# dropbox/rust-brotli

Measured on AMD Instinct MI355X. Metric: compress MB/s at q5 lgwin22, higher is better.
Workload: dtype u8; 1 GPU; 64 MiB synthetic English-like text per GPU, quality=5, lgwin=22, one-shot BrotliEncoderCompress (H6), input and stream resident in HBM; input_bytes_total=67108864, compressed_bytes=16370400

## Files before the change

### rust-brotli_amd/csrc/encoder.cpp

```cpp
#include "encoder.h"
#include "timeline.h"

#include <math.h>
#include <string.h>

#include <algorithm>
#include <chrono>
#include <stdexcept>

#include "device_api.h"
#include "host_entropy.h"
#include "lz77_stage.h"
#include "metablock_api.h"
#include "metablock_device.h"
#include "metablock_hq.h"
#include "metablock_items.h"

namespace brotli_mi355x {

namespace {

struct DevMem {
  DevBlocks blocks;
  static constexpr size_t kArenaBytes = (size_t)4 << 20, kSmall = (size_t)256 << 10;
  uint8_t* arena = nullptr;
  size_t arena_used = kArenaBytes;
  template <typename T>
  T* alloc(size_t count) {
    const size_t bytes = (count * sizeof(T) + 64 + 255) & ~(size_t)255;
    if (bytes > kSmall) return blocks.zeroed<T>(bytes);
    if (arena_used + bytes > kArenaBytes) {
      arena = blocks.zeroed<uint8_t>(kArenaBytes);
      arena_used = 0;
    }
    T* p = (T*)(arena + arena_used);
    arena_used += bytes;
    return p;
  }
};

struct BitPiece {
  uint64_t pos;
  uint32_t nbits;
  uint32_t pad;
  uint64_t bits;
};

struct HostBits {
  uint64_t pos = 0;
  std::vector<BitPiece> pieces;
  void put(uint32_t nbits, uint64_t bits) {
    if (nbits == 0) return;
    pieces.push_back({pos, nbits, 0, bits});
    pos += nbits;
  }
  void jump_to_byte_boundary() { pos = (pos + 7) & ~(uint64_t)7; }
};

void WriteMetadataMetaBlock(const EncoderParams& p, HostBits* hb) {
  uint8_t b128[10];
  size_t count = 0;
  uint64_t value = p.size_hint;
  for (size_t index = 0; index < 10; ++index) {
    b128[index] = (uint8_t)(value & 0x7f);
    value >>= 7;
    count = index + 1;
    if (value != 0) {
      b128[index] |= 0x80;
    } else {
      break;
    }
  }
// ... 640 lines not shown
          j.out_cost = mm.alloc<float>(n + 2);
          j.cluster_size = mm.alloc<uint32_t>(n + 8);
          j.clusters = mm.alloc<uint32_t>(n + 8);
          j.symbols = mm.alloc<uint32_t>(n + 8);
          j.new_index = mm.alloc<uint32_t>(n + 8);
          j.batch_count = mm.alloc<uint32_t>(n / kHqBatch + 8);
          j.reindex_data = mm.alloc<uint32_t>(re * j.len + 8);
          j.reindex_total = mm.alloc<uint32_t>(re + 8);
          j.reindex_cost = mm.alloc<float>(re + 8);
          j.pairs = mm.alloc<HqPair>(std::max<size_t>(kHqBatchPairs, 64 * n) + 2);
          cjobs.push_back(j);
        }
      }
      dev_h2d(B.descs, descs.data(), n_mb * sizeof(MbDesc));
      mb_hq_context_histograms(B);
      HqClusterJob* cjobs_dev = mm.alloc<HqClusterJob>(cjobs.size() + 1);
      dev_h2d(cjobs_dev, cjobs.data(), cjobs.size() * sizeof(HqClusterJob));
      std::vector<HqBatchRef> cbatch_refs;
      for (uint32_t ji = 0; ji < cjobs.size(); ++ji)
        for (uint32_t b = 0; b * kHqBatch < cjobs[ji].in_size; ++b) cbatch_refs.push_back({ji, b});
      HqBatchRef* cbatch_refs_dev = mm.alloc<HqBatchRef>(cbatch_refs.size() + 1);
      dev_h2d(cbatch_refs_dev, cbatch_refs.data(), cbatch_refs.size() * sizeof(HqBatchRef));
      mb_hq_cluster_histograms(B, cjobs_dev, (uint32_t)cjobs.size(), cbatch_refs_dev, (uint32_t)cbatch_refs.size());
      dev_d2h(results.data(), B.results, n_mb * sizeof(MbResult));
      for (uint32_t m = 0; m < n_mb; ++m) results[m].num_histos[kSplitCommand] = results[m].num_types[kSplitCommand];
      dev_h2d(B.results, results.data(), n_mb * sizeof(MbResult));
      stats.ms_phase[3] += clk.lap(prof, "hq-context-maps");
    } else {
      if (p.disable_literal_context_modeling == 0 && p.quality >= 5) {
        uint32_t* stats_dev = mm.alloc<uint32_t>((size_t)n_mb * kContextStatsWords);
        mb_context_stats(B, stats_dev);
        std::vector<uint32_t> cs((size_t)n_mb * kContextStatsWords);
        dev_d2h(cs.data(), stats_dev, cs.size() * 4);
        for (uint32_t m = 0; m < n_mb; ++m) {
          if (descs[m].uncompressed) continue;
          DecideContexts(cs.data() + (size_t)m * kContextStatsWords, p.quality, p.size_hint, descs[m].end - descs[m].start,
                         &descs[m].num_contexts, &descs[m].context_map_id);
        }
      }
      uint32_t gran_total[3] = {0, 0, 0}, row_total[3] = {0, 0, 0}, block_total[3] = {0, 0, 0}, histo_total[3] = {0, 0, 0};
      for (uint32_t m = 0; m < n_mb; ++m) {
        MbDesc& d = descs[m];
        d.n_symbols[0] = d.n_lits;
        d.n_symbols[1] = d.n_cmds;
        d.n_symbols[2] = d.n_dists;
        for (uint32_t k = 0; k < 3; ++k) {
          const uint32_t gl = kGranuleLen[k];
          const uint32_t nc = k == 0 ? d.num_contexts : 1;
          d.granule_base[k] = gran_total[k];
          d.n_granules[k] = d.uncompressed ? 0 : (d.n_symbols[k] + gl - 1) / gl;
          d.gran_row_base[k] = row_total[k];
          d.block_base[k] = block_total[k];
          d.max_blocks[k] = d.n_symbols[k] / gl + 1;
          const uint32_t max_types = (k == 0 && nc > 1) ? 256 / nc : 256;
          d.histo_base[k] = histo_total[k];
          d.max_histos[k] = std::min(d.max_blocks[k], max_types + 1) * nc;
          gran_total[k] += d.n_granules[k];
          row_total[k] += d.n_granules[k] * nc;
          block_total[k] += d.max_blocks[k] + 1;
          histo_total[k] += d.max_histos[k];
        }
      }
      std::vector<uint32_t> gran_mb_host[3];
      for (uint32_t k = 0; k < 3; ++k) {
        gran_mb_host[k].resize(gran_total[k] + 1);
        for (uint32_t m = 0; m < n_mb; ++m)
// ... 72 lines not shown
        if (is_last) {
          bits.put(1, 1);
          bits.put(1, 1);
          bits.jump_to_byte_boundary();
        }
      } else {
        const uint64_t start_bit = bits.pos;
        mb_out_bit[m] = start_bit;
        const uint64_t body_bits = body_off[m + 1] - body_off[m];
        bits.pos += results[m].header_bits + body_bits;
        if (is_last) bits.jump_to_byte_boundary();
        if ((uint64_t)bytes + 4 + (start_bit >> 3) < (bits.pos >> 3)) {
          fallback = (int)m;
          break;
        }
      }
      if (actual_last != is_last) WriteEmptyLastBlocks(p, &bits);
    }
    if (fallback >= 0) {
      lz.ForceUncompressed((uint32_t)fallback);
      stats.fallback_retries++;
      continue;
    }
    if (req.finish && lz.needs_empty_last()) WriteEmptyLastBlocks(p, &bits);
    if (!req.finish && !partial) WriteOpenTail(req, &bits);
    const size_t all_bytes = (size_t)((bits.pos + 7) >> 3);
    const uint32_t tail_nbits = partial ? (uint32_t)(bits.pos & 7) : 0u;
    const size_t total_bytes = tail_nbits ? all_bytes - 1 : all_bytes;
    const size_t out_words = all_bytes / 8 + 4;
    B.out_words = mm.alloc<uint64_t>(out_words);
    if (!all_raw) {
      dev_h2d(B.mb_out_bit, mb_out_bit.data(), (n_mb + 1) * 8);
      mb_emit(B);
    }
    {
      std::vector<MbBitCopy> headers;
      for (uint32_t m = 0; m < n_mb; ++m)
        if (!descs[m].uncompressed) headers.push_back({mb_out_bit[m], (uint64_t)m * B.header_stride, results[m].header_bits});
      std::vector<MbRawCopy> raws;
      for (const RawCopy& rc : copies) raws.push_back({rc.dst_byte, rc.src_pos, rc.bytes});
      std::vector<MbBitPiece> pieces;
      for (const BitPiece& bp : bits.pieces) pieces.push_back({bp.pos, bp.nbits, 0, bp.bits});
      const size_t bytes = headers.size() * sizeof(MbBitCopy) + raws.size() * sizeof(MbRawCopy) + pieces.size() * sizeof(MbBitPiece);
      if (bytes != 0) {
        std::vector<uint8_t> blob(bytes);
        uint8_t* at = blob.data();
        memcpy(at, headers.data(), headers.size() * sizeof(MbBitCopy));
        at += headers.size() * sizeof(MbBitCopy);
        memcpy(at, raws.data(), raws.size() * sizeof(MbRawCopy));
        at += raws.size() * sizeof(MbRawCopy);
        memcpy(at, pieces.data(), pieces.size() * sizeof(MbBitPiece));
        uint8_t* blob_dev = mm.alloc<uint8_t>(bytes + 64);
        dev_h2d(blob_dev, blob.data(), bytes);
        const MbBitCopy* headers_dev = (const MbBitCopy*)blob_dev;
        const MbRawCopy* raws_dev = (const MbRawCopy*)(blob_dev + headers.size() * sizeof(MbBitCopy));
        const MbBitPiece* pieces_dev = (const MbBitPiece*)(blob_dev + headers.size() * sizeof(MbBitCopy) + raws.size() * sizeof(MbRawCopy));
        for (size_t i = 0; i < headers.size(); i += 32768) mb_copy_bits_batch(B.out_words, B.header_words, headers_dev + i, (uint32_t)std::min<size_t>(32768, headers.size() - i));
        for (size_t i = 0; i < raws.size(); i += 32768) mb_raw_copies((uint8_t*)B.out_words, text, raws_dev + i, (uint32_t)std::min<size_t>(32768, raws.size() - i));
        mb_place_pieces(B.out_words, pieces_dev, (uint32_t)pieces.size());
        dev_sync();
      }
    }
    stats.ms_phase[7] += clk.lap(prof, "mb7");
    if (req.direct_out) {
      if (total_bytes > req.direct_capacity) throw std::runtime_error("brotli_mi355x: output buffer too small");
      if (req.direct_out_on_device) {
// ... 102 lines not shown
```

### rust-brotli_amd/csrc/metablock_api.h

```cpp
#ifndef BROTLI_MI355X_METABLOCK_API_H_
#define BROTLI_MI355X_METABLOCK_API_H_

#include <stddef.h>
#include <stdint.h>

#include "metablock_types.h"

namespace brotli_mi355x {

struct MbBuffers;
struct HqSplitJob;
struct HqClusterJob;
struct HqBatchRef;

static constexpr uint32_t kContextStatsWords = 512;

struct CodeJob {
  uint32_t kind;
  uint32_t row_index;
  uint32_t num_distance_symbols;
  uint32_t mode;
};

size_t mb_scan_scratch_bytes(size_t n);
void mb_command_scans(const MbBuffers& B, void* scan_scratch);
void mb_gather_at_metablock_starts(const MbBuffers& B, const uint32_t* src, uint32_t* out_dev);
void mb_gather_bytes(const uint8_t* text, const uint32_t* positions_dev, uint32_t n, uint8_t* out_dev);
void mb_literal_map(const MbBuffers& B);
void mb_context_stats(const MbBuffers& B, uint32_t* stats_dev);
void mb_granule_histograms(const MbBuffers& B);
void mb_split_chains(const MbBuffers& B, bool wide = false);
void mb_build_codes(const MbBuffers& B, const CodeJob* jobs_dev, uint32_t n_jobs);
void mb_write_headers(const MbBuffers& B);
void mb_symbol_bits(const MbBuffers& B, void* scan_scratch);
void mb_emit(const MbBuffers& B);
void mb_copy_bits(uint64_t* out, uint64_t dst_bit, const uint64_t* src, uint64_t nbits);
struct MbBitCopy {
  uint64_t dst_bit, src_word, nbits;
};
void mb_copy_bits_batch(uint64_t* out, const uint64_t* src_words, const MbBitCopy* items_dev, uint32_t n);
struct MbBitPiece {
  uint64_t pos;
  uint32_t nbits, pad;
  uint64_t bits;
};
void mb_place_pieces(uint64_t* out, const MbBitPiece* pieces_dev, uint32_t n);
struct MbRawCopy {
  uint64_t dst_byte;
  uint32_t src_pos, bytes;
};
void mb_raw_copies(uint8_t* out_bytes, const uint8_t* text, const MbRawCopy* items_dev, uint32_t n);

void mb_hq_utf8_census(const MbBuffers& B);
void mb_hq_distance_params(const MbBuffers& B);
void mb_hq_gather_symbols(const MbBuffers& B);
void mb_hq_find_blocks(const MbBuffers& B, HqSplitJob* jobs_dev, uint32_t n_jobs);
void mb_hq_cluster_blocks(const MbBuffers& B, const HqSplitJob* jobs_dev, uint32_t n_jobs, const HqBatchRef* batches_dev, uint32_t n_batches);
void mb_hq_context_histograms(const MbBuffers& B);
void mb_hq_cluster_histograms(const MbBuffers& B, const HqClusterJob* jobs_dev, uint32_t n_jobs, const HqBatchRef* batches_dev,
                              uint32_t n_batches);

}
#endif
```

### rust-brotli_amd/csrc/metablock_device.h

```cpp
#ifndef BROTLI_MI355X_METABLOCK_DEVICE_H_
#define BROTLI_MI355X_METABLOCK_DEVICE_H_

#include "lz77_chain.h"
#include "metablock_types.h"

namespace brotli_mi355x {

struct BitSink {
  uint64_t* words;
  uint64_t pos;
  BR_DEV void put(uint32_t n_bits, uint64_t bits) {
    if (n_bits == 0) return;
    const uint32_t sh = (uint32_t)(pos & 63u);
    uint64_t* w = words + (pos >> 6);
    w[0] |= bits << sh;
    if (sh + n_bits > 64) w[1] |= bits >> (64 - sh);
    pos += n_bits;
  }
};

#if defined(BR_CODES_PROFILE) && !defined(BROTLI_HOST_EMU)
extern __device__ unsigned long long g_codes_prof[32];
struct CodesPhaseClock {
  unsigned long long last;
  BR_DEV CodesPhaseClock() : last(__builtin_readcyclecounter()) {}
  BR_DEV void mark(int phase) {
    const unsigned long long now = __builtin_readcyclecounter();
    if ((threadIdx.x & 63u) == 0) {
      atomicAdd(&g_codes_prof[phase], now - last);
      atomicMax(&g_codes_prof[16 + phase], now - last);
    }
    last = __builtin_readcyclecounter();
  }
};
#define BR_PHASE_CLOCK() CodesPhaseClock br_phase_clock
#define BR_PHASE(k) br_phase_clock.mark(k)
#else
#define BR_PHASE_CLOCK()
#define BR_PHASE(k)
#endif

struct HuffmanTree {
  uint32_t total_count_;
  int16_t index_left_;
  int16_t index_right_or_value_;
};

BR_DEV bool br_set_depth(int p0, HuffmanTree* pool, uint8_t* depth, int max_depth) {
  int stack[16];
  int level = 0;
  int p = p0;
  stack[0] = -1;
  for (;;) {
    if (pool[p].index_left_ >= 0) {
      level++;
      if (level > max_depth) return false;
      stack[level] = pool[p].index_right_or_value_;
      p = pool[p].index_left_;
      continue;
    } else {
      depth[pool[p].index_right_or_value_] = (uint8_t)level;
    }
    while (level >= 0 && stack[level] == -1) level--;
    if (level < 0) return true;
    p = stack[level];
    stack[level] = -1;
  }
}

BR_DEV bool br_sort_cmp(const HuffmanTree& v0, const HuffmanTree& v1) {
  if (v0.total_count_ != v1.total_count_) return v0.total_count_ < v1.total_count_;
  return v0.index_right_or_value_ > v1.index_right_or_value_;
// ... 898 lines not shown
    out.put(1, use_rle ? 1 : 0);
    if (use_rle) out.put(4, max_run_length_prefix - 1);
  }
  br_build_and_store_huffman_tree(histogram, num_clusters + max_run_length_prefix, num_clusters + max_run_length_prefix, sc,
                                  depths, bits, out);
  for (uint32_t i = 0; i < num_rle_symbols; ++i) {
    const uint32_t rle_symbol = rle_symbols[i] & kSymbolMask;
    const uint32_t extra_bits_val = rle_symbols[i] >> 9;
    out.put(depths[rle_symbol], bits[rle_symbol]);
    if (rle_symbol > 0 && rle_symbol <= max_run_length_prefix) out.put(rle_symbol, extra_bits_val);
  }
  out.put(1, 1);
}

BR_DEV void br_store_compressed_meta_block_header(bool is_final_block, uint32_t length, BitSink& out) {
  out.put(1, is_final_block ? 1 : 0);
  if (is_final_block) out.put(1, 0);
  const uint32_t lg = length == 1 ? 1 : br_log2_floor_nonzero(length - 1) + 1;
  const uint32_t mnibbles = (lg < 16 ? 16 : lg + 3) / 4;
  out.put(2, mnibbles - 4);
  out.put(mnibbles * 4, length - 1);
  if (!is_final_block) out.put(1, 0);
}

BR_DEV uint32_t br_context(const uint8_t* utf8_lut, const uint8_t* signed_lut, uint8_t p1, uint8_t p2, uint32_t mode) {
  switch (mode) {
    case 3: return (uint32_t)((signed_lut[p1] << 3) + signed_lut[p2]);
    case 2: return (uint32_t)(utf8_lut[p1] | utf8_lut[256 + p2]);
    case 1: return (uint32_t)(p1 >> 2);
    default: return (uint32_t)(p1 & 0x3f);
  }
}

BR_DEV uint32_t br_static_context_map(uint32_t map_id, uint32_t context) {
  const uint8_t kComplex[64] = {11, 11, 12, 12, 0, 0, 0, 0, 1, 1, 9, 9, 2, 2, 2, 2, 1, 1, 1, 1, 8, 3, 3, 3, 1, 1, 1, 1, 2, 2, 2, 2,
                                8,  4,  4,  4,  8, 7, 4, 4, 8, 0, 0, 0, 3, 3, 3, 3, 5, 5, 10, 5, 5, 5, 10, 5, 6, 6, 6, 6, 6, 6, 6, 6};
  switch (map_id) {
    case 1: return (context == 2 || context == 3) ? 1u : 0u;
    case 2: return context < 2 ? 1u : (context < 4 ? 2u : 0u);
    case 3: return kComplex[context];
    default: return 0;
  }
}

BR_DEV uint32_t br_copy_len_code(const Command& c) {
  const uint32_t modifier = c.copy_len_ >> 25;
  const int32_t delta = (int32_t)(int8_t)(uint8_t)(modifier | ((modifier & 0x40) << 1));
  return (uint32_t)((int32_t)(c.copy_len_ & 0x01ffffffu) + delta);
}

BR_DEV uint32_t br_ins_base(uint32_t code) {
  const uint32_t k[24] = {0, 1, 2, 3, 4, 5, 6, 8, 10, 14, 18, 26, 34, 50, 66, 98, 130, 194, 322, 578, 1090, 2114, 6210, 22594};
  return k[code];
}
BR_DEV uint32_t br_ins_extra(uint32_t code) {
  const uint8_t k[24] = {0, 0, 0, 0, 0, 0, 1, 1, 2, 2, 3, 3, 4, 4, 5, 5, 6, 7, 8, 9, 10, 12, 14, 24};
  return k[code];
}
BR_DEV uint32_t br_copy_base(uint32_t code) {
  const uint32_t k[24] = {2, 3, 4, 5, 6, 7, 8, 9, 10, 12, 14, 18, 22, 30, 38, 54, 70, 102, 134, 198, 326, 582, 1094, 2118};
  return k[code];
}
BR_DEV uint32_t br_copy_extra(uint32_t code) {
  const uint8_t k[24] = {0, 0, 0, 0, 0, 0, 0, 0, 1, 1, 2, 2, 3, 3, 4, 4, 5, 5, 6, 7, 8, 9, 10, 24};
  return k[code];
}

BR_DEV uint64_t br_command_extra_bits(const Command& cmd, uint32_t* nbits) {
  const uint32_t copylen_code = br_copy_len_code(cmd);
// ... 14 lines not shown
```

### rust-brotli_amd/csrc/metablock_items.h

```cpp
#ifndef BROTLI_MI355X_METABLOCK_ITEMS_H_
#define BROTLI_MI355X_METABLOCK_ITEMS_H_

#include "metablock_fast.h"

#if defined(BROTLI_HOST_EMU)
#define BR_TID 0
#define BR_NT 1
#define BR_ATOMIC_ADD_U32(p, v) (*(p) += (v))
#define BR_ATOMIC_OR_U64(p, v) (*(p) |= (v))
#else
#define BR_TID ((int)threadIdx.x)
#define BR_NT ((int)blockDim.x)
#define BR_ATOMIC_ADD_U32(p, v) atomicAdd((p), (v))
#define BR_ATOMIC_OR_U64(p, v) atomicOr((unsigned long long*)(p), (unsigned long long)(v))
#endif

namespace brotli_mi355x {

struct MbBuffers {
  const uint8_t* text;
  const Command* cmds;
  uint32_t n_cmds, n_lits, n_dists, n_mb;
  uint32_t text_base;
  MbDesc* descs;
// ... 439 lines not shown
  const uint32_t row = kRowLen[kind];
  B.tree_nbits[kind][row_index] =
      mb_build_code_core(kind, num_distance_symbols, B.histo[kind] + (size_t)row_index * row, B.depth[kind] + (size_t)row_index * row,
                         B.bits[kind] + (size_t)row_index * row, B.tree_bits[kind] + (size_t)row_index * kTreeBitsWords, sc, false, mode);
}

BR_DEV void mb_append_bits(BitSink& out, const uint64_t* words, uint32_t nbits) {
  uint32_t i = 0;
  while (nbits >= 32) {
    out.put(32, (words[i >> 1] >> ((i & 1) * 32)) & 0xffffffffull);
    nbits -= 32;
    i++;
  }
  if (nbits) out.put(nbits, (words[i >> 1] >> ((i & 1) * 32)) & ((1ull << nbits) - 1));
}

struct MbSplitPrepared {
  uint32_t histograms[3][258 + 26];
  BlockSplitCode code[3];
};
BR_DEV void mb_item_write_header(const MbBuffers& B, uint32_t m, HuffmanScratch* sc, uint64_t* staging = nullptr, MbSplitPrepared* prepared = nullptr) {
  const MbDesc d = B.descs[m];
  MbResult& r = B.results[m];
  if (d.uncompressed) {
    r.header_bits = 0;
    return;
  }
  uint64_t* words = staging ? staging : B.header_words + (size_t)m * B.header_stride;
  if (!staging)
    for (uint32_t i = 0; i < B.header_stride; ++i) words[i] = 0;
  BitSink out;
  out.words = words;
  out.pos = 0;
  br_store_compressed_meta_block_header(d.is_last != 0, d.end - d.start, out);
  BlockSplitCode own_code;
  for (uint32_t kind = 0; kind < 3; ++kind) {
    BlockSplitCode& code = prepared ? prepared->code[kind] : own_code;
    for (int i = 0; i < 258; ++i) {
      code.type_depths[i] = 0;
      code.type_bits[i] = 0;
    }
    for (int i = 0; i < 26; ++i) {
      code.length_depths[i] = 0;
      code.length_bits[i] = 0;
    }
    br_build_and_store_block_split_code(B.block_types[kind] + d.block_base[kind], B.block_lengths[kind] + d.block_base[kind],
                                        r.num_blocks[kind], r.num_types[kind], sc, &code,
                                        B.switch_bits[kind] + d.block_base[kind], B.switch_nbits[kind] + d.block_base[kind], out,
                                        prepared ? prepared->histograms[kind] : nullptr);
  }
  out.put(2, d.dist_postfix_bits);
  out.put(4, d.num_direct_distance_codes >> d.dist_postfix_bits);
  for (uint32_t i = 0; i < r.num_types[kSplitLiteral]; ++i) out.put(2, d.context_mode);
  if (d.hq) {
    uint32_t* scratch = B.ctxmap_scratch + (size_t)m * (2 * 256 * 64);
    br_encode_context_map(B.hq_ctx_map[0] + d.hq_ctx_map_base[0], r.num_types[kSplitLiteral] << 6, r.num_histos[kSplitLiteral], scratch, sc, out);
    br_encode_context_map(B.hq_ctx_map[1] + d.hq_ctx_map_base[1], r.num_types[kSplitDistance] << 2, r.num_histos[kSplitDistance], scratch, sc, out);
  } else {
    if (d.num_contexts <= 1) {
      br_store_trivial_context_map(r.num_histos[kSplitLiteral], 6, sc, out);
    } else {
      uint32_t* cm = B.ctxmap_scratch + (size_t)m * (2 * 256 * 64);
      const uint32_t n = r.num_types[kSplitLiteral] << 6;
      for (uint32_t i = 0; i < r.num_types[kSplitLiteral]; ++i)
        for (uint32_t j = 0; j < 64; ++j) cm[(i << 6) + j] = i * d.num_contexts + br_static_context_map(d.context_map_id, j);
      br_encode_context_map(cm, n, r.num_histos[kSplitLiteral], cm + 256 * 64, sc, out);
    }
    br_store_trivial_context_map(r.num_histos[kSplitDistance], 2, sc, out);
  }
  for (uint32_t kind = 0; kind < 3; ++kind) {
    for (uint32_t i = 0; i < r.num_histos[kind]; ++i) {
      const uint32_t row_index = d.histo_base[kind] + i;
      mb_append_bits(out, B.tree_bits[kind] + (size_t)row_index * kTreeBitsWords, B.tree_nbits[kind][row_index]);
    }
  }
  r.header_bits = (uint32_t)out.pos;
}

BR_DEV uint32_t mb_find_by_lit(const MbBuffers& B, uint32_t i) {
  uint32_t lo = 0, hi = B.n_mb;
  while (hi - lo > 1) {
    const uint32_t mid = (lo + hi) >> 1;
    if (B.descs[mid].lit_base <= i) {
      lo = mid;
    } else {
      hi = mid;
    }
  }
  while (lo + 1 < B.n_mb && B.descs[lo].n_lits == 0 && B.descs[lo + 1].lit_base <= i) lo++;
  return lo;
}
BR_DEV uint32_t mb_find_by_cmd(const MbBuffers& B, uint32_t c) {
  uint32_t lo = 0, hi = B.n_mb;
  while (hi - lo > 1) {
    const uint32_t mid = (lo + hi) >> 1;
    if (B.descs[mid].cmd_offset <= c) {
      lo = mid;
    } else {
      hi = mid;
    }
  }
  return lo;
}

struct SymbolCode {
  uint64_t bits;
  uint32_t nbits;
};
// ... 102 lines not shown
  const size_t ix = ((size_t)d.histo_base[kSplitDistance] + histo) * kNumDistanceHistoSymbols + dist_code;
  sc.bits |= (uint64_t)B.bits[kSplitDistance][ix] << sc.nbits;
  sc.nbits += B.depth[kSplitDistance][ix];
  return sc;
}

BR_DEV void mb_item_literal_nbits(const MbBuffers& B, uint32_t i) { B.lit_nbits[i] = mb_literal_code(B, i).nbits; }

BR_DEV void mb_item_command_nbits(const MbBuffers& B, uint32_t c) {
  const uint32_t m = mb_find_by_cmd(B, c);
  const MbDesc& d = B.descs[m];
  if (d.uncompressed) {
    B.cmd_nbits[c] = 0;
    B.cmd_own_bits[c] = 0;
    return;
  }
  const Command cmd = B.cmds[c];
  SymbolCode own = mb_command_code(B, c, d, m);
  const SymbolCode dist = mb_distance_code(B, c, d, m);
  const uint32_t dist_extra_n = br_command_has_distance(cmd) ? (uint32_t)(cmd.dist_prefix_ >> 10) : 0;
  const uint32_t lit_bits = B.lit_nbits[B.cmd_lit_start[c + 1]] - B.lit_nbits[B.cmd_lit_start[c]];
  B.cmd_own_bits[c] = own.nbits;
  B.cmd_nbits[c] = own.nbits + lit_bits + dist.nbits + dist_extra_n;
}

BR_DEV void mb_put_bits_atomic(uint64_t* words, uint64_t pos, uint32_t nbits, uint64_t bits) {
  if (nbits == 0) return;
  const uint32_t sh = (uint32_t)(pos & 63u);
  uint64_t* w = words + (pos >> 6);
  BR_ATOMIC_OR_U64(w, bits << sh);
  if (sh + nbits > 64) BR_ATOMIC_OR_U64(w + 1, bits >> (64 - sh));
}

BR_DEV void mb_item_emit_command(const MbBuffers& B, uint32_t c) {
  const uint32_t m = mb_find_by_cmd(B, c);
  const MbDesc& d = B.descs[m];
  if (d.uncompressed) return;
  const Command cmd = B.cmds[c];
  const uint64_t base = B.mb_out_bit[m] + B.results[m].header_bits + (B.cmd_nbits[c] - B.cmd_nbits[d.cmd_offset]);
  {
    SymbolCode sc;
    sc.bits = 0;
    sc.nbits = 0;
    const uint32_t local = c - d.cmd_offset;
    bool at_switch;
    const uint32_t blk = mb_block_of(B, d, m, kSplitCommand, local, &at_switch);
    const uint32_t type = B.block_types[kSplitCommand][d.block_base[kSplitCommand] + blk];
    if (at_switch) {
      sc.bits = B.switch_bits[kSplitCommand][d.block_base[kSplitCommand] + blk];
      sc.nbits = B.switch_nbits[kSplitCommand][d.block_base[kSplitCommand] + blk];
    }
    uint64_t pos = base;
    mb_put_bits_atomic(B.out_words, pos, sc.nbits, sc.bits);
    pos += sc.nbits;
    const size_t ix = ((size_t)d.histo_base[kSplitCommand] + type) * kNumCommandSymbols + cmd.cmd_prefix_;
    mb_put_bits_atomic(B.out_words, pos, B.depth[kSplitCommand][ix], B.bits[kSplitCommand][ix]);
    pos += B.depth[kSplitCommand][ix];
    uint32_t en;
    const uint64_t eb = br_command_extra_bits(cmd, &en);
    mb_put_bits_atomic(B.out_words, pos, en, eb);
  }
  if (br_command_has_distance(cmd)) {
    const uint32_t lit_bits = B.lit_nbits[B.cmd_lit_start[c + 1]] - B.lit_nbits[B.cmd_lit_start[c]];
    uint64_t pos = base + B.cmd_own_bits[c] + lit_bits;
    const SymbolCode dc = mb_distance_code(B, c, d, m);
    mb_put_bits_atomic(B.out_words, pos, dc.nbits, dc.bits);
    pos += dc.nbits;
    mb_put_bits_atomic(B.out_words, pos, (uint32_t)(cmd.dist_prefix_ >> 10), cmd.dist_extra_);
  }
}

BR_DEV void mb_item_emit_literal(const MbBuffers& B, uint32_t i) {
  const uint32_t m = mb_find_by_lit(B, i);
  const MbDesc& d = B.descs[m];
  if (d.uncompressed) return;
  const uint32_t c = B.lit_cmd[i];
  const uint64_t pos = B.mb_out_bit[m] + B.results[m].header_bits + (B.cmd_nbits[c] - B.cmd_nbits[d.cmd_offset]) + B.cmd_own_bits[c] +
                       (B.lit_nbits[i] - B.lit_nbits[B.cmd_lit_start[c]]);
  const SymbolCode sc = mb_literal_code(B, i);
  mb_put_bits_atomic(B.out_words, pos, sc.nbits, sc.bits);
}

BR_DEV void mb_item_copy_bits_word(uint64_t* out, uint64_t dst_bit, const uint64_t* src, uint64_t nbits, uint64_t w) {
  const uint64_t first = w * 64;
  if (first >= nbits) return;
  uint32_t n = nbits - first >= 64 ? 64u : (uint32_t)(nbits - first);
  uint64_t v = src[w];
  if (n < 64) v &= (1ull << n) - 1;
  mb_put_bits_atomic(out, dst_bit + first, n, v);
}

}
#endif
```

### rust-brotli_amd/csrc/metablock_kernels.hip

```cpp
#include <hip/hip_runtime.h>

#include "device_api.h"
#include "device_scan.h"
#include "metablock_api.h"
#include "metablock_hq.h"

namespace brotli_mi355x {

size_t mb_scan_scratch_bytes(size_t n) { return scan_scratch_words(n) * 4 + 256; }

template <typename F>
__global__ __launch_bounds__(256) void k_for_each(uint32_t n, F f) {
  const uint32_t i = blockIdx.x * blockDim.x + threadIdx.x;
  if (i < n) f(i);
}
template <typename F>
static void for_each(uint32_t n, F f) {
  if (n == 0) return;
  hipLaunchKernelGGL(k_for_each<F>, dim3((n + 255) / 256), dim3(256), 0, BR_STREAM, n, f);
}

void mb_gather_at_metablock_starts(const MbBuffers& B, const uint32_t* src, uint32_t* out_dev) {
  const MbBuffers b = B;
  for_each(b.n_mb + 1, [b, src, out_dev] __device__(uint32_t m) { out_dev[m] = src[m < b.n_mb ? b.descs[m].cmd_offset : b.n_cmds]; });
  HIP_CHECK(hipGetLastError());
}

void mb_gather_bytes(const uint8_t* text, const uint32_t* positions_dev, uint32_t n, uint8_t* out_dev) {
  for_each(n, [text, positions_dev, out_dev] __device__(uint32_t i) {
    const uint32_t p = positions_dev[i];
    out_dev[i] = p == 0xffffffffu ? (uint8_t)0 : text[p];
  });
  HIP_CHECK(hipGetLastError());
}

void mb_command_scans(const MbBuffers& B, void* scan_scratch) {
  const MbBuffers b = B;
  for_each(b.n_cmds, [b] __device__(uint32_t c) { mb_item_command_counts(b, c); });
  dev_memset(b.cmd_lit_start + b.n_cmds, 0, 4);
  dev_memset(b.cmd_pos + b.n_cmds, 0, 4);
  dev_memset(b.cmd_dist_index + b.n_cmds, 0, 4);
  exclusive_scan_u32(b.cmd_lit_start, b.n_cmds + 1, (uint32_t*)scan_scratch);
  exclusive_scan_u32(b.cmd_pos, b.n_cmds + 1, (uint32_t*)scan_scratch);
  exclusive_scan_u32(b.cmd_dist_index, b.n_cmds + 1, (uint32_t*)scan_scratch);
  HIP_CHECK(hipGetLastError());
}

void mb_literal_map(const MbBuffers& B) {
  const MbBuffers b = B;
  for_each(b.n_lits, [b] __device__(uint32_t i) { mb_item_literal_map(b, i); });
  HIP_CHECK(hipGetLastError());
}

__global__ __launch_bounds__(256) void k_context_stats(MbBuffers B, uint32_t* stats) {
  __shared__ uint32_t s[kContextStatsWords];
  const uint32_t m = blockIdx.x;
  const MbDesc d = B.descs[m];
  for (uint32_t j = threadIdx.x; j < kContextStatsWords; j += blockDim.x) s[j] = 0;
  __syncthreads();
  const uint32_t length = d.end - d.start;
  const uint32_t n_strides = length >= 64 ? (length - 64) / 4096 + 1 : 0;
  for (uint32_t t = threadIdx.x; t < n_strides; t += blockDim.x) {
    const uint32_t start_pos = d.start + t * 4096;
    const uint8_t* p = B.text + start_pos;
    {
      const int lut[4] = {0, 0, 1, 2};
      int prev = lut[p[0] >> 6] * 3;
      for (uint32_t k = 1; k < 64; ++k) {
        const uint8_t literal = p[k];
        atomicAdd(&s[prev + lut[literal >> 6]], 1u);
        prev = lut[literal >> 6] * 3;
      }
    }
    {
      uint8_t prev2 = p[0], prev1 = p[1];
      for (uint32_t k = 2; k < 64; ++k) {
        const uint8_t literal = p[k];
        const uint32_t context = br_static_context_map(3, br_context(B.utf8_lut, B.signed_lut, prev1, prev2, 2));
        atomicAdd(&s[480], 1u);
        atomicAdd(&s[16 + (literal >> 3)], 1u);
        atomicAdd(&s[48 + context * 32 + (literal >> 3)], 1u);
        prev2 = prev1;
        prev1 = literal;
      }
    }
  }
  __syncthreads();
  for (uint32_t j = threadIdx.x; j < kContextStatsWords; j += blockDim.x) stats[(size_t)m * kContextStatsWords + j] = s[j];
}

void mb_context_stats(const MbBuffers& B, uint32_t* stats_dev) {
  if (B.n_mb == 0) return;
  hipLaunchKernelGGL(k_context_stats, dim3(B.n_mb), dim3(256), 0, BR_STREAM, B, stats_dev);
  HIP_CHECK(hipGetLastError());
}

__global__ __launch_bounds__(256) void k_granule_histograms(MbBuffers B, uint32_t kind) {
  __shared__ uint32_t lds[kMaxStaticContexts * 256];
  mb_item_granule_histogram(B, kind, blockIdx.x, lds);
}

void mb_granule_histograms(const MbBuffers& B) {
  const MbBuffers b = B;
  if (b.n_granules[kSplitLiteral]) hipLaunchKernelGGL(k_granule_histograms, dim3(b.n_granules[kSplitLiteral]), dim3(256), 0, BR_STREAM, b, (uint32_t)kSplitLiteral);
  if (b.n_granules[kSplitCommand]) hipLaunchKernelGGL(k_granule_histograms, dim3(b.n_granules[kSplitCommand]), dim3(256), 0, BR_STREAM, b, (uint32_t)kSplitCommand);
  if (b.n_granules[kSplitDistance]) {
    dev_memset(b.gran_hist[kSplitDistance], 0, (size_t)b.n_granules[kSplitDistance] * kNumDistanceHistoSymbols * 2);
    for_each(b.n_cmds, [b] __device__(uint32_t c) { mb_item_distance_count(b, c); });
  }
  HIP_CHECK(hipGetLastError());
}

__global__ __launch_bounds__(1024) void k_split_chains(MbBuffers B) {
  __shared__ SplitScratch S;
  mb_item_split_chain(B, blockIdx.x / 3, blockIdx.x % 3, S);
}

void mb_split_chains(const MbBuffers& B, bool wide) {
  if (B.n_mb == 0) return;
  hipLaunchKernelGGL(k_split_chains, dim3(B.n_mb * 3), dim3(wide ? 1024 : 256), 0, BR_STREAM, B);
  HIP_CHECK(hipGetLastError());
}

#if defined(BR_CODES_PROFILE)
__device__ unsigned long long g_codes_prof[32];
#endif
__global__ __launch_bounds__(64) void k_build_codes(MbBuffers B, const CodeJob* jobs, uint32_t n_jobs) {
  __shared__ HuffmanScratch sc;
  __shared__ uint32_t h[704];
  __shared__ uint16_t bits[704];
  __shared__ uint8_t depth[704];
  __shared__ uint64_t words[kTreeBitsWords];
  __shared__ uint32_t nbits;
  const uint32_t i = blockIdx.x;
  if (i >= n_jobs) return;
  const CodeJob j = jobs[i];
  const uint32_t row = kRowLen[j.kind];
  uint32_t* gh = B.histo[j.kind] + (size_t)j.row_index * row;
  for (uint32_t k = threadIdx.x; k < row; k += 64) h[k] = gh[k];
  __syncthreads();
  {
    const uint32_t nb = mb_build_code_core(j.kind, j.num_distance_symbols, h, depth, bits, words, &sc, true, j.mode);
    if (threadIdx.x == 0) nbits = nb;
  }
  __syncthreads();
  uint8_t* gd = B.depth[j.kind] + (size_t)j.row_index * row;
  uint16_t* gb = B.bits[j.kind] + (size_t)j.row_index * row;
  uint64_t* gw = B.tree_bits[j.kind] + (size_t)j.row_index * kTreeBitsWords;
  for (uint32_t k = threadIdx.x; k < row; k += 64) {
    gh[k] = h[k];
    gd[k] = depth[k];
    gb[k] = bits[k];
  }
  for (uint32_t k = threadIdx.x; k < kTreeBitsWords; k += 64) gw[k] = words[k];
  if (threadIdx.x == 0) B.tree_nbits[j.kind][j.row_index] = nbits;
}

void mb_build_codes(const MbBuffers& B, const CodeJob* jobs_dev, uint32_t n_jobs) {
  if (n_jobs == 0) return;
// ... 47 lines not shown
      if (i != 0) atomicAdd(&prep.histograms[kind][br_block_type_code_at(types, i)], 1u);
      atomicAdd(&prep.histograms[kind][258 + br_block_length_prefix_code(lengths[i])], 1u);
    }
  }
  __syncthreads();
  if (threadIdx.x == 0) {
    mb_item_write_header(B, m, &sc_lds, stage, &prep);
    s_bits = B.results[m].header_bits;
  }
  __syncthreads();
  for (uint32_t kind = 0; kind < 3; ++kind) {
    if (B.results[m].num_types[kind] <= 1) continue;
    const uint8_t* types = B.block_types[kind] + d.block_base[kind];
    const uint32_t* lengths = B.block_lengths[kind] + d.block_base[kind];
    uint64_t* switch_bits = B.switch_bits[kind] + d.block_base[kind];
    uint8_t* switch_nbits = B.switch_nbits[kind] + d.block_base[kind];
    const uint32_t nb = B.results[m].num_blocks[kind];
    for (uint32_t i = 1 + threadIdx.x; i < nb; i += 64) {
      uint32_t nbits;
      switch_bits[i] = br_block_switch_bits(prep.code[kind], br_block_type_code_at(types, i), lengths[i], false, &nbits);
      switch_nbits[i] = (uint8_t)nbits;
    }
  }
  if (in_lds) {
    const uint32_t words = (s_bits + 63) / 64 + 1;
    for (uint32_t i = threadIdx.x; i < words && i < kLdsWords; i += 64) global_words[i] = lw[i];
  }
}

void mb_write_headers(const MbBuffers& B) {
  if (B.n_mb == 0) return;
  hipLaunchKernelGGL(k_write_headers, dim3(B.n_mb), dim3(64), 0, BR_STREAM, B);
  HIP_CHECK(hipGetLastError());
}

void mb_symbol_bits(const MbBuffers& B, void* scan_scratch) {
  const MbBuffers b = B;
  for_each(b.n_lits, [b] __device__(uint32_t i) { mb_item_literal_nbits(b, i); });
  dev_memset(b.lit_nbits + b.n_lits, 0, 4);
  exclusive_scan_u32(b.lit_nbits, b.n_lits + 1, (uint32_t*)scan_scratch);
  for_each(b.n_cmds, [b] __device__(uint32_t c) { mb_item_command_nbits(b, c); });
  dev_memset(b.cmd_nbits + b.n_cmds, 0, 4);
  exclusive_scan_u32(b.cmd_nbits, b.n_cmds + 1, (uint32_t*)scan_scratch);
  HIP_CHECK(hipGetLastError());
}

void mb_emit(const MbBuffers& B) {
  const MbBuffers b = B;
  for_each(b.n_cmds, [b] __device__(uint32_t c) { mb_item_emit_command(b, c); });
  for_each(b.n_lits, [b] __device__(uint32_t i) { mb_item_emit_literal(b, i); });
  HIP_CHECK(hipGetLastError());
}

__global__ __launch_bounds__(256) void k_hq_utf8_census(MbBuffers B) {
  __shared__ HqCensusScratch S;
  if (!B.descs[blockIdx.x].uncompressed) hq_item_utf8_census(B, blockIdx.x, S);
}
void mb_hq_utf8_census(const MbBuffers& B) {
  if (B.n_mb == 0) return;
  hipLaunchKernelGGL(k_hq_utf8_census, dim3(B.n_mb), dim3(256), 0, BR_STREAM, B);
  HIP_CHECK(hipGetLastError());
}
__global__ __launch_bounds__(64) void k_hq_distance_params(MbBuffers B) {
  __shared__ HqWaveScratch S;
  hq_item_distance_params(B, blockIdx.x, S);
}
void mb_hq_distance_params(const MbBuffers& B) {
  if (B.n_mb == 0) return;
  hipLaunchKernelGGL(k_hq_distance_params, dim3(B.n_mb), dim3(64), 0, BR_STREAM, B);
  HIP_CHECK(hipGetLastError());
}
void mb_hq_gather_symbols(const MbBuffers& B) {
  const MbBuffers b = B;
  for_each(b.n_lits, [b] __device__(uint32_t i) { hq_item_literal_symbol(b, i); });
  for_each(b.n_cmds, [b] __device__(uint32_t c) { hq_item_command_symbols(b, c); });
  HIP_CHECK(hipGetLastError());
}
__global__ __launch_bounds__(64) void k_hq_find_blocks(EntropyTables et, HqSplitJob* jobs) {
  __shared__ HqWaveScratch S;
  hq_item_find_blocks(et, jobs[blockIdx.x], S);
}
// ... 112 lines not shown
```

Baseline: 4142 MB/s.

## Parallelize context stats across chunks and batch emission atomics in LDS windows

The context-statistics kernel now spreads each meta-block's strides over 64 blocks and wave lanes. It uses ballot-based counting and shuffles instead of per-thread serial loops, and merges the partial results into global memory with atomics. The symbol emission path stages each wave's bit writes in a shared-memory window of words and then flushes them with one atomic OR per word, instead of issuing a global atomic for every piece. Env-gated self-tests and optional header-phase profiling counters are also added. The risks are extra grid overhead for small meta-blocks, and global fallback atomics when a wave's bits do not fit in its window.

```diff
diff --git a/rust-brotli_amd/csrc/encoder.cpp b/rust-brotli_amd/csrc/encoder.cpp
--- a/rust-brotli_amd/csrc/encoder.cpp
+++ b/rust-brotli_amd/csrc/encoder.cpp
@@ -38,6 +38,46 @@
     return p;
   }
 };
+
+void SelfTestContextStats(const uint8_t* text_dev, const std::vector<MbDesc>& descs, const std::vector<uint32_t>& rows) {
+  uint8_t utf8[512];
+  dev_d2h(utf8, dev_tables().utf8_context_lookup, sizeof(utf8));
+  std::vector<uint8_t> bytes;
+  for (size_t m = 0; m < descs.size(); ++m) {
+    uint32_t s[kContextStatsWords] = {0};
+    const uint32_t length = descs[m].end - descs[m].start;
+    const uint32_t n_strides = length >= 64 ? (length - 64) / 4096 + 1 : 0;
+    bytes.resize(length);
+    if (n_strides) dev_d2h(bytes.data(), text_dev + descs[m].start, length);
+    for (uint32_t t = 0; t < n_strides; ++t) {
+      const uint8_t* p = bytes.data() + (size_t)t * 4096;
+      const uint32_t lut[4] = {0, 0, 1, 2};
+      for (uint32_t k = 1; k < 64; ++k) s[lut[p[k - 1] >> 6] * 3 + lut[p[k] >> 6]]++;
+      for (uint32_t k = 2; k < 64; ++k) {
+        const uint32_t context = kStaticContextMapComplexUTF8[utf8[p[k - 1]] | utf8[256 + p[k - 2]]];
+        s[480]++;
+        s[16 + (p[k] >> 3)]++;
+        s[48 + context * 32 + (p[k] >> 3)]++;
+      }
+    }
+    for (uint32_t j = 0; j < kContextStatsWords; ++j)
+      if (rows[m * kContextStatsWords + j] != s[j])
+        throw std::runtime_error("selftest: context statistics of meta-block " + std::to_string(m) + " differ at word " + std::to_string(j));
+  }
+}
+
+void SelfTestEmit(const MbBuffers& B, size_t out_words) {
+#if !defined(BROTLI_HOST_EMU)
+  DevBlocks blocks;
+  uint64_t* again = blocks.zeroed<uint64_t>(out_words * 8);
+  mb_emit_piecewise(B, again);
+  std::vector<uint64_t> a(out_words), b(out_words);
+  dev_d2h(a.data(), B.out_words, out_words * 8);
+  dev_d2h(b.data(), again, out_words * 8);
+  for (size_t i = 0; i < out_words; ++i)
+    if (a[i] != b[i]) throw std::runtime_error("selftest: mb_emit differs from the piecewise emission at word " + std::to_string(i));
+#endif
+}
 
 struct BitPiece {
   uint64_t pos;
@@ -744,6 +784,7 @@
         mb_context_stats(B, stats_dev);
         std::vector<uint32_t> cs((size_t)n_mb * kContextStatsWords);
         dev_d2h(cs.data(), stats_dev, cs.size() * 4);
+        if (getenv("BROTLI_MI355X_SELFTEST")) SelfTestContextStats(text, descs, cs);
         for (uint32_t m = 0; m < n_mb; ++m) {
           if (descs[m].uncompressed) continue;
           DecideContexts(cs.data() + (size_t)m * kContextStatsWords, p.quality, p.size_hint, descs[m].end - descs[m].start,
@@ -882,6 +923,7 @@
     if (!all_raw) {
       dev_h2d(B.mb_out_bit, mb_out_bit.data(), (n_mb + 1) * 8);
       mb_emit(B);
+      if (getenv("BROTLI_MI355X_SELFTEST")) SelfTestEmit(B, out_words);
     }
     {
       std::vector<MbBitCopy> headers;
diff --git a/rust-brotli_amd/csrc/metablock_api.h b/rust-brotli_amd/csrc/metablock_api.h
--- a/rust-brotli_amd/csrc/metablock_api.h
+++ b/rust-brotli_amd/csrc/metablock_api.h
@@ -34,6 +34,7 @@
 void mb_write_headers(const MbBuffers& B);
 void mb_symbol_bits(const MbBuffers& B, void* scan_scratch);
 void mb_emit(const MbBuffers& B);
+void mb_emit_piecewise(const MbBuffers& B, uint64_t* out_words);
 void mb_copy_bits(uint64_t* out, uint64_t dst_bit, const uint64_t* src, uint64_t nbits);
 struct MbBitCopy {
   uint64_t dst_bit, src_word, nbits;
diff --git a/rust-brotli_amd/csrc/metablock_device.h b/rust-brotli_amd/csrc/metablock_device.h
--- a/rust-brotli_amd/csrc/metablock_device.h
+++ b/rust-brotli_amd/csrc/metablock_device.h
@@ -20,7 +20,7 @@
 };
 
 #if defined(BR_CODES_PROFILE) && !defined(BROTLI_HOST_EMU)
-extern __device__ unsigned long long g_codes_prof[32];
+static __device__ unsigned long long g_codes_prof[32];
 struct CodesPhaseClock {
   unsigned long long last;
   BR_DEV CodesPhaseClock() : last(__builtin_readcyclecounter()) {}
@@ -35,9 +35,24 @@
 };
 #define BR_PHASE_CLOCK() CodesPhaseClock br_phase_clock
 #define BR_PHASE(k) br_phase_clock.mark(k)
+static __device__ unsigned long long g_header_prof[16];
+struct HeaderPhaseClock {
+  unsigned long long last;
+  BR_DEV HeaderPhaseClock() : last(__builtin_readcyclecounter()) {}
+  BR_DEV void mark(int phase) {
+    const unsigned long long now = __builtin_readcyclecounter();
+    atomicAdd(&g_header_prof[phase], now - last);
+    atomicMax(&g_header_prof[8 + phase], now - last);
+    last = __builtin_readcyclecounter();
+  }
+};
+#define BR_HEADER_PHASE_CLOCK() HeaderPhaseClock br_header_clock
+#define BR_HEADER_PHASE(k) br_header_clock.mark(k)
 #else
 #define BR_PHASE_CLOCK()
 #define BR_PHASE(k)
+#define BR_HEADER_PHASE_CLOCK()
+#define BR_HEADER_PHASE(k)
 #endif
 
 struct HuffmanTree {
@@ -1002,9 +1017,11 @@
   }
 }
 
+static constexpr uint8_t kStaticContextMapComplexUTF8[64] = {11, 11, 12, 12, 0, 0, 0, 0, 1, 1, 9,  9, 2, 2, 2,  2, 1, 1, 1, 1, 8, 3,
+                                                             3,  3,  1,  1,  1, 1, 2, 2, 2, 2, 8,  4, 4, 4, 8,  7, 4, 4, 8, 0, 0, 0,
+                                                             3,  3,  3,  3,  5, 5, 10, 5, 5, 5, 10, 5, 6, 6, 6, 6, 6, 6, 6, 6};
 BR_DEV uint32_t br_static_context_map(uint32_t map_id, uint32_t context) {
-  const uint8_t kComplex[64] = {11, 11, 12, 12, 0, 0, 0, 0, 1, 1, 9, 9, 2, 2, 2, 2, 1, 1, 1, 1, 8, 3, 3, 3, 1, 1, 1, 1, 2, 2, 2, 2,
-                                8,  4,  4,  4,  8, 7, 4, 4, 8, 0, 0, 0, 3, 3, 3, 3, 5, 5, 10, 5, 5, 5, 10, 5, 6, 6, 6, 6, 6, 6, 6, 6};
+  const uint8_t* kComplex = kStaticContextMapComplexUTF8;
   switch (map_id) {
     case 1: return (context == 2 || context == 3) ? 1u : 0u;
     case 2: return context < 2 ? 1u : (context < 4 ? 2u : 0u);
diff --git a/rust-brotli_amd/csrc/metablock_items.h b/rust-brotli_amd/csrc/metablock_items.h
--- a/rust-brotli_amd/csrc/metablock_items.h
+++ b/rust-brotli_amd/csrc/metablock_items.h
@@ -495,6 +495,7 @@
   BitSink out;
   out.words = words;
   out.pos = 0;
+  BR_HEADER_PHASE_CLOCK();
   br_store_compressed_meta_block_header(d.is_last != 0, d.end - d.start, out);
   BlockSplitCode own_code;
   for (uint32_t kind = 0; kind < 3; ++kind) {
@@ -512,6 +513,7 @@
                                         B.switch_bits[kind] + d.block_base[kind], B.switch_nbits[kind] + d.block_base[kind], out,
                                         prepared ? prepared->histograms[kind] : nullptr);
   }
+  BR_HEADER_PHASE(0);
   out.put(2, d.dist_postfix_bits);
   out.put(4, d.num_direct_distance_codes >> d.dist_postfix_bits);
   for (uint32_t i = 0; i < r.num_types[kSplitLiteral]; ++i) out.put(2, d.context_mode);
@@ -531,12 +533,14 @@
     }
     br_store_trivial_context_map(r.num_histos[kSplitDistance], 2, sc, out);
   }
+  BR_HEADER_PHASE(1);
   for (uint32_t kind = 0; kind < 3; ++kind) {
     for (uint32_t i = 0; i < r.num_histos[kind]; ++i) {
       const uint32_t row_index = d.histo_base[kind] + i;
       mb_append_bits(out, B.tree_bits[kind] + (size_t)row_index * kTreeBitsWords, B.tree_nbits[kind][row_index]);
     }
   }
+  BR_HEADER_PHASE(2);
   r.header_bits = (uint32_t)out.pos;
 }
 
@@ -705,12 +709,24 @@
   if (sh + nbits > 64) BR_ATOMIC_OR_U64(w + 1, bits >> (64 - sh));
 }
 
-BR_DEV void mb_item_emit_command(const MbBuffers& B, uint32_t c) {
+struct MbAtomicSink {
+  uint64_t* words;
+  BR_DEV void put(uint64_t pos, uint32_t nbits, uint64_t bits) const { mb_put_bits_atomic(words, pos, nbits, bits); }
+};
+
+BR_DEV bool mb_command_base(const MbBuffers& B, uint32_t c, uint32_t* m_out, uint64_t* base) {
   const uint32_t m = mb_find_by_cmd(B, c);
   const MbDesc& d = B.descs[m];
-  if (d.uncompressed) return;
+  if (d.uncompressed) return false;
+  *m_out = m;
+  *base = B.mb_out_bit[m] + B.results[m].header_bits + (B.cmd_nbits[c] - B.cmd_nbits[d.cmd_offset]);
+  return true;
+}
+
+template <typename Sink>
+BR_DEV void mb_emit_command_pieces(const MbBuffers& B, uint32_t c, uint32_t m, uint64_t base, const Sink& sink) {
+  const MbDesc& d = B.descs[m];
   const Command cmd = B.cmds[c];
-  const uint64_t base = B.mb_out_bit[m] + B.results[m].header_bits + (B.cmd_nbits[c] - B.cmd_nbits[d.cmd_offset]);
   {
     SymbolCode sc;
     sc.bits = 0;
@@ -724,35 +740,51 @@
       sc.nbits = B.switch_nbits[kSplitCommand][d.block_base[kSplitCommand] + blk];
     }
     uint64_t pos = base;
-    mb_put_bits_atomic(B.out_words, pos, sc.nbits, sc.bits);
+    sink.put(pos, sc.nbits, sc.bits);
     pos += sc.nbits;
     const size_t ix = ((size_t)d.histo_base[kSplitCommand] + type) * kNumCommandSymbols + cmd.cmd_prefix_;
-    mb_put_bits_atomic(B.out_words, pos, B.depth[kSplitCommand][ix], B.bits[kSplitCommand][ix]);
+    sink.put(pos, B.depth[kSplitCommand][ix], B.bits[kSplitCommand][ix]);
     pos += B.depth[kSplitCommand][ix];
     uint32_t en;
     const uint64_t eb = br_command_extra_bits(cmd, &en);
-    mb_put_bits_atomic(B.out_words, pos, en, eb);
+    sink.put(pos, en, eb);
   }
   if (br_command_has_distance(cmd)) {
     const uint32_t lit_bits = B.lit_nbits[B.cmd_lit_start[c + 1]] - B.lit_nbits[B.cmd_lit_start[c]];
     uint64_t pos = base + B.cmd_own_bits[c] + lit_bits;
     const SymbolCode dc = mb_distance_code(B, c, d, m);
-    mb_put_bits_atomic(B.out_words, pos, dc.nbits, dc.bits);
+    sink.put(pos, dc.nbits, dc.bits);
     pos += dc.nbits;
-    mb_put_bits_atomic(B.out_words, pos, (uint32_t)(cmd.dist_prefix_ >> 10), cmd.dist_extra_);
-  }
-}
-
-BR_DEV void mb_item_emit_literal(const MbBuffers& B, uint32_t i) {
+    sink.put(pos, (uint32_t)(cmd.dist_prefix_ >> 10), cmd.dist_extra_);
+  }
+}
+
+template <typename Sink>
+BR_DEV void mb_item_emit_command(const MbBuffers& B, uint32_t c, const Sink& sink) {
+  uint32_t m;
+  uint64_t base;
+  if (mb_command_base(B, c, &m, &base)) mb_emit_command_pieces(B, c, m, base, sink);
+}
+BR_DEV void mb_item_emit_command(const MbBuffers& B, uint32_t c) { mb_item_emit_command(B, c, MbAtomicSink{B.out_words}); }
+
+BR_DEV bool mb_literal_base(const MbBuffers& B, uint32_t i, uint64_t* pos) {
   const uint32_t m = mb_find_by_lit(B, i);
   const MbDesc& d = B.descs[m];
-  if (d.uncompressed) return;
+  if (d.uncompressed) return false;
   const uint32_t c = B.lit_cmd[i];
-  const uint64_t pos = B.mb_out_bit[m] + B.results[m].header_bits + (B.cmd_nbits[c] - B.cmd_nbits[d.cmd_offset]) + B.cmd_own_bits[c] +
-                       (B.lit_nbits[i] - B.lit_nbits[B.cmd_lit_start[c]]);
+  *pos = B.mb_out_bit[m] + B.results[m].header_bits + (B.cmd_nbits[c] - B.cmd_nbits[d.cmd_offset]) + B.cmd_own_bits[c] +
+         (B.lit_nbits[i] - B.lit_nbits[B.cmd_lit_start[c]]);
+  return true;
+}
+
+template <typename Sink>
+BR_DEV void mb_item_emit_literal(const MbBuffers& B, uint32_t i, const Sink& sink) {
+  uint64_t pos;
+  if (!mb_literal_base(B, i, &pos)) return;
   const SymbolCode sc = mb_literal_code(B, i);
-  mb_put_bits_atomic(B.out_words, pos, sc.nbits, sc.bits);
-}
+  sink.put(pos, sc.nbits, sc.bits);
+}
+BR_DEV void mb_item_emit_literal(const MbBuffers& B, uint32_t i) { mb_item_emit_literal(B, i, MbAtomicSink{B.out_words}); }
 
 BR_DEV void mb_item_copy_bits_word(uint64_t* out, uint64_t dst_bit, const uint64_t* src, uint64_t nbits, uint64_t w) {
   const uint64_t first = w * 64;
diff --git a/rust-brotli_amd/csrc/metablock_kernels.hip b/rust-brotli_amd/csrc/metablock_kernels.hip
--- a/rust-brotli_amd/csrc/metablock_kernels.hip
+++ b/rust-brotli_amd/csrc/metablock_kernels.hip
@@ -52,46 +52,64 @@
   HIP_CHECK(hipGetLastError());
 }
 
+static constexpr uint32_t kStatsChunks = 64;
 __global__ __launch_bounds__(256) void k_context_stats(MbBuffers B, uint32_t* stats) {
   __shared__ uint32_t s[kContextStatsWords];
-  const uint32_t m = blockIdx.x;
+  const uint32_t m = blockIdx.y;
   const MbDesc d = B.descs[m];
-  for (uint32_t j = threadIdx.x; j < kContextStatsWords; j += blockDim.x) s[j] = 0;
-  __syncthreads();
   const uint32_t length = d.end - d.start;
   const uint32_t n_strides = length >= 64 ? (length - 64) / 4096 + 1 : 0;
-  for (uint32_t t = threadIdx.x; t < n_strides; t += blockDim.x) {
-    const uint32_t start_pos = d.start + t * 4096;
-    const uint8_t* p = B.text + start_pos;
-    {
-      const int lut[4] = {0, 0, 1, 2};
-      int prev = lut[p[0] >> 6] * 3;
-      for (uint32_t k = 1; k < 64; ++k) {
-        const uint8_t literal = p[k];
-        atomicAdd(&s[prev + lut[literal >> 6]], 1u);
-        prev = lut[literal >> 6] * 3;
+  const uint32_t wave = threadIdx.x >> 6, lane = threadIdx.x & 63, n_waves = kStatsChunks * 4;
+  if (blockIdx.x * 4 >= n_strides) return;
+  for (uint32_t j = threadIdx.x; j < kContextStatsWords; j += blockDim.x) s[j] = 0;
+  __syncthreads();
+  const uint8_t* text = B.text + d.start + lane;
+  constexpr uint32_t kBatch = 4;
+  for (uint32_t t0 = blockIdx.x * 4 + wave; t0 < n_strides; t0 += n_waves * kBatch) {
+    uint32_t bytes[kBatch];
+    for (uint32_t u = 0; u < kBatch; ++u) {
+      const uint32_t t = t0 + u * n_waves;
+      bytes[u] = t < n_strides ? text[(size_t)t * 4096] : 0u;
+    }
+    for (uint32_t u = 0; u < kBatch; ++u) {
+      if (t0 + u * n_waves >= n_strides) break;
+      const uint32_t literal = bytes[u];
+      const uint32_t prev1 = (uint32_t)__shfl_up((int)literal, 1, 64), prev2 = (uint32_t)__shfl_up((int)literal, 2, 64);
+      {
+        const uint32_t lut = 0x90u;
+        const uint32_t bin = ((lut >> ((prev1 >> 6) * 2)) & 3u) * 3u + ((lut >> ((literal >> 6) * 2)) & 3u);
+        uint32_t mine = 0;
+        for (uint32_t b = 0; b < 9; ++b) {
+          const uint32_t count = (uint32_t)__popcll(__ballot(lane >= 1 && bin == b));
+          if (lane == b) mine = count;
+        }
+        if (mine) atomicAdd(&s[lane], mine);
       }
+      if (lane >= 2) {
+        const uint32_t context = br_static_context_map(3, br_context(B.utf8_lut, B.signed_lut, (uint8_t)prev1, (uint8_t)prev2, 2));
+        atomicAdd(&s[48 + context * 32 + (literal >> 3)], 1u);
+      }
+      if (lane == 0) atomicAdd(&s[480], 62u);
     }
-    {
-      uint8_t prev2 = p[0], prev1 = p[1];
-      for (uint32_t k = 2; k < 64; ++k) {
-        const uint8_t literal = p[k];
-        const uint32_t context = br_static_context_map(3, br_context(B.utf8_lut, B.signed_lut, prev1, prev2, 2));
-        atomicAdd(&s[480], 1u);
-        atomicAdd(&s[16 + (literal >> 3)], 1u);
-        atomicAdd(&s[48 + context * 32 + (literal >> 3)], 1u);
-        prev2 = prev1;
-        prev1 = literal;
-      }
-    }
-  }
-  __syncthreads();
-  for (uint32_t j = threadIdx.x; j < kContextStatsWords; j += blockDim.x) stats[(size_t)m * kContextStatsWords + j] = s[j];
+  }
+  __syncthreads();
+  uint32_t* row = stats + (size_t)m * kContextStatsWords;
+  for (uint32_t j = threadIdx.x; j < kContextStatsWords; j += blockDim.x) {
+    uint32_t v = s[j];
+    if (j >= 16 && j < 48)
+      for (uint32_t c = 0; c < 13; ++c) v += s[48 + c * 32 + (j - 16)];
+    if (v) atomicAdd(&row[j], v);
+  }
 }
 
 void mb_context_stats(const MbBuffers& B, uint32_t* stats_dev) {
   if (B.n_mb == 0) return;
-  hipLaunchKernelGGL(k_context_stats, dim3(B.n_mb), dim3(256), 0, BR_STREAM, B, stats_dev);
+  for (uint32_t first = 0; first < B.n_mb; first += 32768) {
+    MbBuffers b = B;
+    b.descs += first;
+    const uint32_t n = B.n_mb - first < 32768 ? B.n_mb - first : 32768;
+    hipLaunchKernelGGL(k_context_stats, dim3(kStatsChunks, n), dim3(256), 0, BR_STREAM, b, stats_dev + (size_t)first * kContextStatsWords);
+  }
   HIP_CHECK(hipGetLastError());
 }
 
@@ -122,9 +140,6 @@
   HIP_CHECK(hipGetLastError());
 }
 
-#if defined(BR_CODES_PROFILE)
-__device__ unsigned long long g_codes_prof[32];
-#endif
 __global__ __launch_bounds__(64) void k_build_codes(MbBuffers B, const CodeJob* jobs, uint32_t n_jobs) {
   __shared__ HuffmanScratch sc;
   __shared__ uint32_t h[704];
@@ -238,6 +253,17 @@
   if (B.n_mb == 0) return;
   hipLaunchKernelGGL(k_write_headers, dim3(B.n_mb), dim3(64), 0, BR_STREAM, B);
   HIP_CHECK(hipGetLastError());
+#if defined(BR_CODES_PROFILE)
+  {
+    unsigned long long h[16];
+    HIP_CHECK(hipStreamSynchronize(BR_STREAM));
+    HIP_CHECK(hipMemcpyFromSymbol(h, HIP_SYMBOL(g_header_prof), sizeof(h)));
+    fprintf(stderr, "header profile (%u meta-blocks), cycles sum / slowest meta-block: block-split codes %llu / %llu, context maps %llu / %llu, trees %llu / %llu\n",
+            B.n_mb, h[0], h[8], h[1], h[9], h[2], h[10]);
+    unsigned long long z[16] = {0};
+    HIP_CHECK(hipMemcpyToSymbol(HIP_SYMBOL(g_header_prof), z, sizeof(z)));
+  }
+#endif
 }
 
 void mb_symbol_bits(const MbBuffers& B, void* scan_scratch) {
@@ -251,8 +277,75 @@
   HIP_CHECK(hipGetLastError());
 }
 
+template <uint32_t kWords>
+struct MbWindowSink {
+  uint64_t* words;
+  unsigned long long* window;
+  uint64_t first_word;
+  __device__ __forceinline__ void put(uint64_t pos, uint32_t nbits, uint64_t bits) const {
+    if (nbits == 0) return;
+    const uint32_t sh = (uint32_t)(pos & 63u);
+    const uint64_t at = (pos >> 6) - first_word;
+    const bool two = sh + nbits > 64;
+    if (at < kWords && (!two || at + 1 < kWords)) {
+      atomicOr(window + at, (unsigned long long)(bits << sh));
+      if (two) atomicOr(window + at + 1, (unsigned long long)(bits >> (64 - sh)));
+    } else {
+      mb_put_bits_atomic(words, pos, nbits, bits);
+    }
+  }
+};
+
+static constexpr uint32_t kEmitCommandWindow = 128;
+static constexpr uint32_t kEmitLiteralWindow = 64;
+
+template <uint32_t kWords, typename First, typename Emit>
+__device__ __forceinline__ void mb_emit_wave(const MbBuffers& B, uint32_t n, unsigned long long* windows, First first, Emit emit) {
+  const uint32_t lane = threadIdx.x & 63u;
+  unsigned long long* window = windows + (threadIdx.x >> 6) * kWords;
+  for (uint32_t j = lane; j < kWords; j += 64) window[j] = 0;
+  const uint32_t i = blockIdx.x * blockDim.x + threadIdx.x;
+  uint64_t bit = 0;
+  const bool mine = i < n && first(i, &bit);
+  const unsigned long long emitting = __ballot(mine);
+  uint64_t first_word = 0;
+  if (emitting) first_word = (uint64_t)__shfl((unsigned long long)(bit >> 6), __ffsll(emitting) - 1, 64);
+  __syncthreads();
+  if (mine) emit(i, bit, MbWindowSink<kWords>{B.out_words, window, first_word});
+  __syncthreads();
+  for (uint32_t j = lane; j < kWords; j += 64) {
+    const unsigned long long v = window[j];
+    if (v) atomicOr((unsigned long long*)B.out_words + first_word + j, v);
+  }
+}
+
+__global__ __launch_bounds__(256) void k_emit_commands(MbBuffers B) {
+  __shared__ unsigned long long windows[4 * kEmitCommandWindow];
+  uint32_t m = 0;
+  mb_emit_wave<kEmitCommandWindow>(
+      B, B.n_cmds, windows, [&](uint32_t c, uint64_t* bit) { return mb_command_base(B, c, &m, bit); },
+      [&](uint32_t c, uint64_t bit, const MbWindowSink<kEmitCommandWindow>& sink) { mb_emit_command_pieces(B, c, m, bit, sink); });
+}
+
+__global__ __launch_bounds__(256) void k_emit_literals(MbBuffers B) {
+  __shared__ unsigned long long windows[4 * kEmitLiteralWindow];
+  mb_emit_wave<kEmitLiteralWindow>(
+      B, B.n_lits, windows, [&](uint32_t i, uint64_t* bit) { return mb_literal_base(B, i, bit); },
+      [&](uint32_t i, uint64_t bit, const MbWindowSink<kEmitLiteralWindow>& sink) {
+        const SymbolCode sc = mb_literal_code(B, i);
+        sink.put(bit, sc.nbits, sc.bits);
+      });
+}
+
 void mb_emit(const MbBuffers& B) {
-  const MbBuffers b = B;
+  if (B.n_cmds) hipLaunchKernelGGL(k_emit_commands, dim3((B.n_cmds + 255) / 256), dim3(256), 0, BR_STREAM, B);
+  if (B.n_lits) hipLaunchKernelGGL(k_emit_literals, dim3((B.n_lits + 255) / 256), dim3(256), 0, BR_STREAM, B);
+  HIP_CHECK(hipGetLastError());
+}
+
+void mb_emit_piecewise(const MbBuffers& B, uint64_t* out_words) {
+  MbBuffers b = B;
+  b.out_words = out_words;
   for_each(b.n_cmds, [b] __device__(uint32_t c) { mb_item_emit_command(b, c); });
   for_each(b.n_lits, [b] __device__(uint32_t i) { mb_item_emit_literal(b, i); });
   HIP_CHECK(hipGetLastError());
```

After: 4334 MB/s, median of 6. 4.6% higher.
